# yerfor/Real3DPortrait

Measured on AMD Instinct MI355X. Metric: rendered frames/sec @ 512x512, 48 depth samples, higher is better.
Workload: dtype f32 operands as fp16 hi + lo, fp32 accumulate (SR precision 'f16mx' = the library default, superresolution.DEFAULT_SR_PRECISION; the fp32-class f16x3 is `alt_f16x3`): in block0.conv1, block1.conv0 and block1.conv1 hi*hi runs on the f16 MFMA and the two cross products on the block-scaled 8-bit MFMA

## Files before the change

### real3dportrait_amd/csrc/r3d_render.hip

```cpp

#include "r3d_common.h"
#include "r3d_stamps.h"

namespace r3d {

static constexpr int kC = R3D_FEATURES;
static constexpr int kHid = R3D_HIDDEN;
static constexpr int kOut = R3D_DECODER_OUT;
static constexpr int kWavesPerBlock = 4;

__device__ __forceinline__ void block_absmax_store(float m, float* __restrict__ absmax_part, int block_linear, float* red)
{
#pragma unroll
    for (int d = 32; d >= 1; d >>= 1) m = fmaxf(m, __shfl_xor(m, d));
    const int tid = threadIdx.y * blockDim.x + threadIdx.x, nw = (blockDim.x * blockDim.y) >> 6;
    if ((tid & 63) == 0) red[tid >> 6] = m;
    __syncthreads();
    if (tid == 0) {
        float r = red[0];
        for (int w = 1; w < nw; ++w) r = fmaxf(r, red[w]);
        absmax_part[block_linear] = r;
    }
}

// ... 506 lines not shown
#pragma unroll
    for (int ot = 0; ot < 2; ++ot) {
        uint4 a0 = L.w2f[ot][PP][0][lane], a1 = L.w2f[ot][PP][1][lane];
        const h8 wh = *reinterpret_cast<h8*>(&a0), wl = *reinterpret_cast<h8*>(&a1);
        col[ot] = __builtin_amdgcn_mfma_f32_16x16x32_f16(wl, bh, col[ot], 0, 0, 0);
        col[ot] = __builtin_amdgcn_mfma_f32_16x16x32_f16(wh, bl, col[ot], 0, 0, 0);
        col[ot] = __builtin_amdgcn_mfma_f32_16x16x32_f16(wh, bh, col[ot], 0, 0, 0);
    }
    if (PP == 1) {
        const float ys = L.ys;
        if (ys != 1.0f) {
#pragma unroll
            for (int ot = 0; ot < 2; ++ot)
#pragma unroll
                for (int r = 0; r < 4; ++r) col[ot][r] *= ys;
        }
#pragma unroll
        for (int ot = 0; ot < 2; ++ot)
#pragma unroll
            for (int r = 0; r < 4; ++r)
                col[ot][r] = __builtin_amdgcn_rcpf(1.0f + __builtin_amdgcn_exp2f(-col[ot][r])) * 1.002f - 0.001f;
    }
}

__device__ __forceinline__ void decode_tile(const DecoderLds& L, int lane, const h8 xh, const h8 xl, f32x4 (&col)[2], float& sig)
{
    DecodeState S;
    decode_a(L, lane, xh, xl, S, sig);
    decode_l2<0>(L, lane, S, col);
    decode_l2<1>(L, lane, S, col);
}

template <int CTRL, int ROW_MASK = 0xF>
__device__ __forceinline__ float dpp_f(float old, float x) {
    return __builtin_bit_cast(float, __builtin_amdgcn_update_dpp(__builtin_bit_cast(int, old), __builtin_bit_cast(int, x), CTRL, ROW_MASK, 0xF, false));
}
template <int CTRL, int ROW_MASK = 0xF>
__device__ __forceinline__ int dpp_i(int old, int x) { return __builtin_amdgcn_update_dpp(old, x, CTRL, ROW_MASK, 0xF, false); }
__device__ __forceinline__ float wave_incl_mul(float v, int) {
    v *= dpp_f<0x111>(1.0f, v); v *= dpp_f<0x112>(1.0f, v); v *= dpp_f<0x114>(1.0f, v); v *= dpp_f<0x118>(1.0f, v);
    v *= dpp_f<0x142, 0xA>(1.0f, v); v *= dpp_f<0x143, 0xC>(1.0f, v);
    return v;
}
__device__ __forceinline__ float wave_incl_add(float v, int) {
    v += dpp_f<0x111>(0.0f, v); v += dpp_f<0x112>(0.0f, v); v += dpp_f<0x114>(0.0f, v); v += dpp_f<0x118>(0.0f, v);
    v += dpp_f<0x142, 0xA>(0.0f, v); v += dpp_f<0x143, 0xC>(0.0f, v);
    return v;
}
__device__ __forceinline__ int wave_incl_add_i(int v) {
    v += dpp_i<0x111>(0, v); v += dpp_i<0x112>(0, v); v += dpp_i<0x114>(0, v); v += dpp_i<0x118>(0, v);
    v += dpp_i<0x142, 0xA>(0, v); v += dpp_i<0x143, 0xC>(0, v);
    return v;
}
__device__ __forceinline__ float wave_shift_up1(float v, float first) { return dpp_f<0x138>(first, v); }
__device__ __forceinline__ float lane63(float v) { return __builtin_bit_cast(float, __builtin_amdgcn_readlane(__builtin_bit_cast(int, v), 63)); }
__device__ __forceinline__ float wave_sum(float v) { return lane63(wave_incl_add(v, 0)); }
__device__ __forceinline__ void wave_lds_sync() {
    __builtin_amdgcn_fence(__ATOMIC_ACQ_REL, "wavefront");
    __builtin_amdgcn_wave_barrier();
}

struct XchLds { uint4 v[2][64]; };
__device__ __forceinline__ int gather_q(int lane) { return lane & 3; }
__device__ __forceinline__ int gather_s(int lane) { return lane >> 2; }
__device__ __forceinline__ void gather_to_mfma(XchLds& E, int lane, const float (&X)[8], h8& xh, h8& xl)
{
    split8_bounded(X, xh, xl);
    const int gs = lane >> 2, gq = lane & 3, q = lane >> 4, s = lane & 15;
    const int wi = 16 * gq + (gs ^ (2 * gq)), ri = 16 * q + (s ^ (2 * q));
    E.v[0][wi] = *reinterpret_cast<uint4*>(&xh);
    E.v[1][wi] = *reinterpret_cast<uint4*>(&xl);
    wave_lds_sync();
    uint4 rh = E.v[0][ri], rl = E.v[1][ri];
    wave_lds_sync();
    xh = *reinterpret_cast<h8*>(&rh);
    xl = *reinterpret_cast<h8*>(&rl);
}

template <int NS, int NCD>
struct RayLds {
    float t[NS];
    float sg[NS];
    float ts[NS];
    float ss[NS];
    float wv[NS];
    float om[NS];
    float cdf[NCD];
    int cnt[NS];
};

struct FeatLds { uint4 v[2][2 * 64]; };

typedef __amdgpu_buffer_rsrc_t PlaneRsrc;
template <int NB = 2>
struct TileGather {
    f32x4 lo[NB][4], hi[NB][4];
    float tw[NB][4];
    Tap tq[4];
    float acc[8];
    __device__ __forceinline__ void start(int H, int W, int q, float px, float py, float pz, float scale)
    {
        const float qx = px * scale, qy = py * scale, qz = pz * scale;
        const int pq = q < 2 ? q : 2;
        plane_taps(pq == 2 ? qz : qx, pq == 0 ? qy : (pq == 1 ? qz : qx), H, W, pq * H * W * 8, tq);
#pragma unroll
        for (int k = 0; k < 4; ++k) tq[k].idx *= 16;
    }
    template <int P, int B>
    __device__ __forceinline__ void issue(const PlaneRsrc rsrc, unsigned qoff)
    {
#pragma unroll
        for (int k = 0; k < 4; ++k) {
            const int wbits = __builtin_bit_cast(int, tq[k].w);
            const unsigned off = (unsigned)(P == 0 ? __builtin_amdgcn_mov_dpp(tq[k].idx, 0x00, 0xF, 0xF, true) : P == 1 ? __builtin_amdgcn_mov_dpp(tq[k].idx, 0x55, 0xF, 0xF, true) : __builtin_amdgcn_mov_dpp(tq[k].idx, 0xAA, 0xF, 0xF, true)) + qoff;
            tw[B][k] = __builtin_bit_cast(float, P == 0 ? __builtin_amdgcn_mov_dpp(wbits, 0x00, 0xF, 0xF, true) : P == 1 ? __builtin_amdgcn_mov_dpp(wbits, 0x55, 0xF, 0xF, true) : __builtin_amdgcn_mov_dpp(wbits, 0xAA, 0xF, 0xF, true));
            lo[B][k] = __builtin_bit_cast(f32x4, __builtin_amdgcn_raw_buffer_load_b128(rsrc, (int)off, 0, 0));
            hi[B][k] = __builtin_bit_cast(f32x4, __builtin_amdgcn_raw_buffer_load_b128(rsrc, (int)(off + 16u), 0, 0));
        }
    }
    template <int B>
    __device__ __forceinline__ void pin(f32x4& d0, f32x4& d1)
    {
        asm volatile("" : "+v"(lo[B][0]), "+v"(lo[B][1]), "+v"(lo[B][2]), "+v"(lo[B][3]), "+v"(hi[B][0]), "+v"(hi[B][1]), "+v"(hi[B][2]), "+v"(hi[B][3]),
                          "+v"(d0), "+v"(d1));
    }
    template <int P, int B>
    __device__ __forceinline__ void consume()
    {
        float pa[8];
#pragma unroll
        for (int c = 0; c < 8; ++c) pa[c] = 0.0f;
#pragma unroll
        for (int k = 0; k < 4; ++k) {
            const float w = tw[B][k];
            const f32x4 a4 = lo[B][k], b4 = hi[B][k];
            pa[0] += a4[0] * w; pa[1] += a4[1] * w; pa[2] += a4[2] * w; pa[3] += a4[3] * w;
            pa[4] += b4[0] * w; pa[5] += b4[1] * w; pa[6] += b4[2] * w; pa[7] += b4[3] * w;
        }
#pragma unroll
        for (int c = 0; c < 8; ++c) acc[c] = P == 0 ? pa[c] : acc[c] + pa[c];
    }
    __device__ __forceinline__ void finish(FeatLds& F, int slot, int wi, float xs3)
    {
        float X[8];
#pragma unroll
        for (int c = 0; c < 8; ++c) X[c] = acc[c] * xs3;
        h8 xh, xl;
        split8_bounded(X, xh, xl);
        F.v[0][slot * 64 + wi] = *reinterpret_cast<uint4*>(&xh);
        F.v[1][slot * 64 + wi] = *reinterpret_cast<uint4*>(&xl);
    }
};

template <int NT, int GPF, bool TRI, int NB = 2, typename DepthFn, typename FirstFn>
__device__ __forceinline__ void decode_pass(FeatLds& F, const DecoderLds& dec, const float4* __restrict__ P, int H, int W, int D, int lane,
                                            float ox, float oy, float oz, float dx, float dy, float dz, float scale, float xs3,
                                            DepthFn depth_of, FirstFn first_done, f32x4 (&col0)[NT], f32x4 (&col1)[NT], float (&sig)[NT], f32x4* gp = nullptr)
{
    const int gq = lane & 3, gs = lane >> 2, q = lane >> 4, s = lane & 15;
    const int wi = 16 * gq + (gs ^ (2 * gq)), ri = 16 * q + (s ^ (2 * q));
    const uint64_t pb = (uint64_t)(uintptr_t)P;
    void* pu = reinterpret_cast<void*>((uintptr_t)(((uint64_t)(unsigned)__builtin_amdgcn_readfirstlane((int)(pb >> 32)) << 32) |
                                                   (unsigned)__builtin_amdgcn_readfirstlane((int)(pb & 0xffffffffu))));
    const PlaneRsrc pl = __builtin_amdgcn_make_buffer_rsrc(pu, 0, __builtin_amdgcn_readfirstlane(3 * (TRI ? D : 1) * H * W * 128), 0x00020000);
    const unsigned qoff = 32u * (unsigned)gq;
    TileGather<NB> g;
    auto gather_whole = [&](int t) {
        const float tg = depth_of(t);
        if constexpr (TRI) {
            float X[8]; h8 xh, xl;
            gather_sample<GPF, true>(P, H, W, gq, ox + tg * dx, oy + tg * dy, oz + tg * dz, scale, xs3, X, D);
            split8_bounded(X, xh, xl);
            F.v[0][(t & 1) * 64 + wi] = *reinterpret_cast<uint4*>(&xh); F.v[1][(t & 1) * 64 + wi] = *reinterpret_cast<uint4*>(&xl);
        } else {
            f32x4 z0 = {0.f, 0.f, 0.f, 0.f}, z1 = z0;
            g.start(H, W, gq, ox + tg * dx, oy + tg * dy, oz + tg * dz, scale);
            g.template issue<0, 0>(pl, qoff);
            if constexpr (NB == 2) {
                g.template issue<1, 1>(pl, qoff);
                g.template pin<0>(z0, z1); g.template consume<0, 0>();
                g.template issue<2, 0>(pl, qoff);
                g.template pin<1>(z0, z1); g.template consume<1, 1>();
                g.template pin<0>(z0, z1); g.template consume<2, 0>();
            } else {
                g.template pin<0>(z0, z1); g.template consume<0, 0>();
                g.template issue<1, 0>(pl, qoff);
                g.template pin<0>(z0, z1); g.template consume<1, 0>();
                g.template issue<2, 0>(pl, qoff);
                g.template pin<0>(z0, z1); g.template consume<2, 0>();
            }
            g.finish(F, t & 1, wi, xs3);
        }
    };
    gather_whole(0);
    first_done();
#pragma unroll
    for (int t = 0; t < NT; ++t) {
        wave_lds_sync();
        uint4 rh = F.v[0][(t & 1) * 64 + ri], rl4 = F.v[1][(t & 1) * 64 + ri];
        const h8 xh = *reinterpret_cast<h8*>(&rh), xl = *reinterpret_cast<h8*>(&rl4);
        const bool more = t + 1 < NT;
        DecodeState S;
        f32x4 c2[2];
        if (more && !TRI) {
            const float tg = depth_of(t + 1);
            g.start(H, W, gq, ox + tg * dx, oy + tg * dy, oz + tg * dz, scale);
            g.template issue<0, 0>(pl, qoff);
        }
        __builtin_amdgcn_sched_barrier(0);
        decode_a(dec, lane, xh, xl, S, sig[t]);
        __builtin_amdgcn_sched_barrier(0);
        if (more && !TRI) { g.template pin<0>(S.h[0], S.h[3]); g.template consume<0, 0>(); g.template issue<1, 0>(pl, qoff); }
        __builtin_amdgcn_sched_barrier(0);
        decode_l2<0>(dec, lane, S, c2);
        __builtin_amdgcn_sched_barrier(0);
        if (more && !TRI) { g.template pin<0>(c2[0], c2[1]); g.template consume<1, 0>(); g.template issue<2, 0>(pl, qoff); }
        __builtin_amdgcn_sched_barrier(0);
        decode_l2<1>(dec, lane, S, c2);
        __builtin_amdgcn_sched_barrier(0);
        if (more && !TRI) { g.template pin<0>(c2[0], c2[1]); g.template consume<2, 0>(); g.finish(F, (t + 1) & 1, wi, xs3); }
        if (more && TRI) gather_whole(t + 1);
        if (gp) { gp[(2 * t) * 64] = c2[0]; gp[(2 * t + 1) * 64] = c2[1]; }
        else { col0[t] = c2[0]; col1[t] = c2[1]; }
        __builtin_amdgcn_sched_barrier(0);
    }
}

template <int SLOTS>
__device__ __forceinline__ void march(const float* T, const float* S, float* wv, int n, int lane,
                                      float& wsum, float& dsum)
{
    float carry = 1.0f, ws = 0.0f, ds = 0.0f;
#pragma unroll
    for (int sl = 0; sl < SLOTS; ++sl) {
        const int i = sl * 64 + lane;
        const bool act = i < n - 1;
        const int i0 = act ? i : 0;
        const float t0 = T[i0], t1 = T[i0 + 1], s0 = S[i0], s1 = S[i0 + 1];
        const float delta = t1 - t0;
        const float dmid = (s0 + s1) * 0.5f;
        const float tmid = (t0 + t1) * 0.5f;
        const float sp = softplus20(dmid - 1.0f);
        const float alpha = one_minus_exp_neg(sp * delta);
        const float om1 = act ? (1.0f - alpha + 1e-10f) : 1.0f;
        const float incl = wave_incl_mul(om1, lane);
        const float excl = wave_shift_up1(incl, 1.0f);
        const float w = act ? alpha * (carry * excl) : 0.0f;
        carry *= lane63(incl);
        if (act) wv[i] = w;
        ws += w;
        ds += w * tmid;
    }
    wsum = wave_sum(ws);
    dsum = wave_sum(ds);
}

struct RenderArgs {
    const float4* planes4; int N, H, W, M, D;
    const float* w1; const float* b1; const float* w2; const float* b2;
    const float* origins; const float* dirs;
    const float* cam_c2w; const float* cam_K; int cam_R;
    uint2* split_out; const float* split_scale; size_t split_scale_stride;
    const float* ray_start; const float* ray_end; const uint8_t* valid;
    int* gstate; int nlimit_blocks;
    int Nc, Nf; float scale; int white_back;
    const float* noise_c; const float* u_f; unsigned long long seed;
    const DecFold* fold;
    float* rgb; float* depth; float* wsum; int rgb_cm;
    unsigned long long* clk;
    f32x4* park_g;
};

struct RayIter {
    int strips, n, c, row, sa, sb, sc, R, strip, N, M, col0;
    long long lin, lstride, nrays;
    __device__ __forceinline__ void init(const RenderArgs& a, int R_, int wave)
    {
        const int wv = __builtin_amdgcn_readfirstlane(wave);
        R = R_; N = a.N; M = a.M;
        strips = (R > 0 && (R & 7) == 0 && (gridDim.x & 7) == 0) ? 1 : 0;
        if (strips) {
            const unsigned xcd = blockIdx.x & 7, bx = blockIdx.x >> 3, nbx = gridDim.x >> 3;
            strip = R >> 3; col0 = (int)xcd * strip;
            const unsigned per_img = (unsigned)strip * (unsigned)R;
            const unsigned w0 = bx * kWavesPerBlock + (unsigned)wv, st = nbx * kWavesPerBlock;
            n = (int)(w0 / per_img); const unsigned rem = w0 - (unsigned)n * per_img;
            c = (int)(rem / (unsigned)R); row = (int)(rem - (unsigned)c * (unsigned)R);
            sa = (int)(st / per_img); const unsigned srem = st - (unsigned)sa * per_img;
            sb = (int)(srem / (unsigned)R); sc = (int)(srem - (unsigned)sb * (unsigned)R);
        } else {
            nrays = (long long)a.N * a.M;
            lin = (long long)blockIdx.x * kWavesPerBlock + wv;
            lstride = (long long)gridDim.x * kWavesPerBlock;
        }
    }
    __device__ __forceinline__ bool get(int& ray, int& img) const
    {
        if (strips) { if (n >= N) return false; img = n; ray = n * M + row * R + col0 + c; return true; }
        if (lin >= nrays) return false;
        ray = (int)lin; img = ray / M; return true;
    }
    __device__ __forceinline__ void advance()
    {
        if (strips) {
            row += sc; if (row >= R) { row -= R; ++c; }
            c += sb;   if (c >= strip) { c -= strip; ++n; }
            n += sa;
        } else lin += lstride;
    }
};

template <int NTC, int NTF, int OCC, int GPF, bool TRI = false>
__global__ __launch_bounds__(256, OCC) void render_kernel(RenderArgs a, int R)
{
    constexpr int SLOTS = (16 * (NTC + NTF) + 63) / 64;
    constexpr int CSLOTS = (16 * NTC + 63) / 64;
    constexpr int FSLOTS = NTF > 0 ? (16 * NTF + 63) / 64 : 1;
    typedef RayLds<16 * (NTC + NTF) + 8, 16 * NTC + 8> RayL;
    __shared__ __attribute__((aligned(16))) DecoderLds dec;
    __shared__ __attribute__((aligned(16))) RayL rl[kWavesPerBlock];
    __shared__ __attribute__((aligned(16))) FeatLds feat[kWavesPerBlock];
    constexpr bool PARK = NTF > 0 && NTC <= 3;
    constexpr bool GPARK = NTF > 0 && NTC > 3;
    __shared__ __attribute__((aligned(16))) f32x4 park[PARK ? kWavesPerBlock : 1][PARK ? 2 * NTC : 1][64];

    stage_decoder(dec, a.w1, a.b1, a.w2, a.b2, a.fold);
    __syncthreads();
    const float xs3 = dec.xs3;

    const int lane = threadIdx.x & 63, wave = threadIdx.x >> 6;
    const int q = lane >> 4, s = lane & 15;
    const int gs = gather_s(lane);
    RayL& L = rl[wave];
    FeatLds& F = feat[wave];
    int pmin = 0x7fffffff, pmax = (int)0x80000000, pany = 0;
    for (int b = lane; b < a.nlimit_blocks; b += 64) {
        const int* p = a.gstate + kStateHeader + 3 * b;
        pmin = min(pmin, p[0]); pmax = max(pmax, p[1]); pany |= p[2];
    }
#pragma unroll
    for (int d = 32; d >= 1; d >>= 1) { pmin = min(pmin, __shfl_xor(pmin, d)); pmax = max(pmax, __shfl_xor(pmax, d)); pany |= __shfl_xor(pany, d); }
    const float gmin_start = ord2f(pmin), gmax_start = ord2f(pmax);
    const bool any_valid = pany != 0;
    const int Nc_all = a.Nc;
    float run_min = INFINITY, run_max = -INFINITY;
    R3D_STAMP_DECL;
    int st_rays_ = 0; (void)st_rays_;
    if (blockIdx.x == (gridDim.x >> 1) && threadIdx.x == 0) clk_begin(kernarg_clk<RenderArgs>());

    RayIter it;
    it.init(a, R, wave);
    for (;; it.advance()) {
        typedef const __attribute__((address_space(4))) RenderArgs* KArgs;
        KArgs ap = (KArgs)__builtin_amdgcn_kernarg_segment_ptr();
        asm volatile("" : "+s"(ap));
        const auto& A = *ap;
        const int Nc = NTF > 0 ? A.Nc : Nc_all, Nf = A.Nf, S = Nc + Nf;
        int ray, n;
        if (!it.get(ray, n)) break;
        ++st_rays_;
        R3D_STAMP(7);
        const float4* P = A.planes4 + (size_t)n * 3 * (TRI ? A.D : 1) * A.H * A.W * 8;
        float ox, oy, oz, dx, dy, dz;
        if (A.cam_c2w) {
            float o3[3], d3[3];
            make_ray(A.cam_c2w + 16 * n, A.cam_K + 9 * n, A.cam_R, ray - n * A.M, o3, d3);
            ox = o3[0]; oy = o3[1]; oz = o3[2]; dx = d3[0]; dy = d3[1]; dz = d3[2];
        } else {
            ox = A.origins[3 * (size_t)ray]; oy = A.origins[3 * (size_t)ray + 1]; oz = A.origins[3 * (size_t)ray + 2];
            dx = A.dirs[3 * (size_t)ray]; dy = A.dirs[3 * (size_t)ray + 1]; dz = A.dirs[3 * (size_t)ray + 2];
        }
        float start = A.ray_start[ray], end = A.ray_end[ray];
        if (!A.valid[ray] && any_valid) { start = gmin_start; end = gmax_start; }

        const float span = end - start;
        const float delta = span / (float)(Nc - 1);
        float tc[NTC];
#pragma unroll
        for (int nt = 0; nt < NTC; ++nt) {
            const int k = 16 * nt + s;
            const bool act = k < Nc;
            const float step = (float)k / (float)(Nc - 1);
            float u = 0.0f;
            if (act) u = A.noise_c ? A.noise_c[(size_t)ray * Nc + k] : hash_uniform(A.seed, 0, (uint64_t)ray * Nc + k);
            tc[nt] = act ? (start + step * span) + u * delta : start;
        }
        R3D_STAMP(0);
        f32x4 colc[2][NTC];
        float sigc[NTC];
        f32x4* gpark = nullptr;
        if constexpr (GPARK) gpark = A.park_g + ((size_t)(blockIdx.x * kWavesPerBlock + wave) * (2 * (NTC + NTF))) * 64 + lane;
        {
            if (q == 0) {
#pragma unroll
                for (int nt = 0; nt < NTC; ++nt) {
                    const int k = 16 * nt + s;
                    if (k < Nc) L.t[k] = tc[nt];
                }
            }
            wave_lds_sync();
            auto dof = [&](int t) { const int k = 16 * t + gs; return k < Nc ? L.t[k] : start; };
            decode_pass<NTC, GPF, TRI, (OCC >= 3 ? 1 : 2)>(F, dec, P, A.H, A.W, A.D, lane, ox, oy, oz, dx, dy, dz, A.scale, xs3, dof,
                                                           [&]() { R3D_STAMP(8); }, colc[0], colc[1], sigc, gpark);
        }
        constexpr bool parked = PARK;
        if (parked) {
#pragma unroll
            for (int nt = 0; nt < NTC; ++nt) { park[PARK ? wave : 0][PARK ? 2 * nt : 0][lane] = colc[0][nt]; park[PARK ? wave : 0][PARK ? 2 * nt + 1 : 0][lane] = colc[1][nt]; }
        }

        if (q == 0) {
#pragma unroll
            for (int nt = 0; nt < NTC; ++nt) {
                const int k = 16 * nt + s;
                if (k < Nc) L.sg[k] = sigc[nt];
            }
        }
        wave_lds_sync();
        R3D_STAMP(1);

        float wsum, dsum;
        f32x4 colf[2][NTF > 0 ? NTF : 1];
        bool fine_done = false;
        if constexpr (NTF > 0) { if (Nf > 0) {
            fine_done = true;
            march<CSLOTS>(L.t, L.sg, L.wv, Nc, lane, wsum, dsum);
            wave_lds_sync();
            const int ns = Nc - 3;
            float omega[CSLOTS], tot = 0.0f;
#pragma unroll
            for (int sl = 0; sl < CSLOTS; ++sl) {
                const int i = sl * 64 + lane;
                const bool act = i < ns;
                const int i0 = act ? i : 0;
                const float w0 = L.wv[i0], w1v = L.wv[i0 + 1], w2v = L.wv[i0 + 2];
                const float sv = (fmaxf(w0, w1v) + fmaxf(w1v, w2v)) * 0.5f + 0.01f;
                omega[sl] = act ? sv + 1e-5f : 0.0f;
                tot += omega[sl];
            }
            tot = wave_sum(tot);
            float carry = 0.0f;
            if (lane == 0) L.cdf[0] = 0.0f;
#pragma unroll
            for (int sl = 0; sl < CSLOTS; ++sl) {
                const int i = sl * 64 + lane;
                const float incl = wave_incl_add(omega[sl] / tot, lane);
                if (i < ns) L.cdf[i + 1] = carry + incl;
                carry += lane63(incl);
            }
            wave_lds_sync();
#pragma unroll
            for (int sl = 0; sl < FSLOTS; ++sl) {
                const int j = sl * 64 + lane;
                if (j < Nf) {
                    const float u = A.u_f ? A.u_f[(size_t)ray * Nf + j] : hash_uniform(A.seed, 1, (uint64_t)ray * Nf + j);
                    int lo = 0, hi = ns + 1;
                    while (lo < hi) { const int mid = (lo + hi) >> 1; if (L.cdf[mid] <= u) lo = mid + 1; else hi = mid; }
                    const int below = max(lo - 1, 0), above = min(lo, ns);
                    const float cb = L.cdf[below], ca = L.cdf[above];
                    const float bb = 0.5f * (L.t[below] + L.t[below + 1]);
                    const float ba = 0.5f * (L.t[above] + L.t[above + 1]);
                    float den = ca - cb;
                    if (den < 1e-5f) den = 1.0f;
                    L.t[Nc + j] = bb + (u - cb) / den * (ba - bb);
                }
            }
            wave_lds_sync();
            R3D_STAMP(2);
            float sigf[NTF > 0 ? NTF : 1];
            {
                auto dof = [&](int t) { const int k = 16 * t + gs; return L.t[Nc + (k < Nf ? k : 0)]; };
                decode_pass<(NTF > 0 ? NTF : 1), GPF, TRI, (OCC >= 3 ? 1 : 2)>(F, dec, P, A.H, A.W, A.D, lane, ox, oy, oz, dx, dy, dz, A.scale, xs3, dof,
                                                                             [&]() { R3D_STAMP(9); }, colf[0], colf[1], sigf, GPARK ? gpark + 2 * NTC * 64 : nullptr);
            }
            if (q == 0) {
#pragma unroll
                for (int nt = 0; nt < NTF; ++nt) {
                    const int k = 16 * nt + s;
                    if (k < Nf) L.sg[Nc + k] = sigf[nt];
                }
            }
            wave_lds_sync();
            R3D_STAMP(3);
            int rank[SLOTS];
            bool fast = true;
#pragma unroll
            for (int sl = 0; sl < CSLOTS; ++sl) {
                const int i = sl * 64 + lane;
                const bool act = i < Nc - 1;
                fast = fast && (!act || L.t[act ? i : 0] <= L.t[act ? i + 1 : 0]);
            }
            fast = __all(fast);
            if (fast) {
#pragma unroll
                for (int sl = 0; sl < CSLOTS + 1; ++sl) { const int i = sl * 64 + lane; if (i <= Nc) L.cnt[i] = 0; }
                wave_lds_sync();
                int rf[FSLOTS];
#pragma unroll
                for (int sl = 0; sl < FSLOTS; ++sl) {
                    const int j = sl * 64 + lane;
                    const bool act = j < Nf;
                    const float tj = L.t[Nc + (act ? j : 0)];
                    int lo = 0, hi = Nc;
                    while (lo < hi) { const int mid = (lo + hi) >> 1; if (L.t[mid] <= tj) lo = mid + 1; else hi = mid; }
                    int f = 0;
                    for (int k = 0; k < Nf; ++k) f += (L.t[Nc + k] < tj) ? 1 : 0;
                    rf[sl] = lo + f;
                    if (act) atomicAdd(&L.cnt[lo], 1);
                }
                wave_lds_sync();
                int carry = 0;
                int rc[CSLOTS];
#pragma unroll
                for (int sl = 0; sl < CSLOTS; ++sl) {
                    const int i = sl * 64 + lane;
                    int v = i < Nc ? L.cnt[i] : 0;
                    v = wave_incl_add_i(v);
                    rc[sl] = i + carry + v;
                    carry += __builtin_amdgcn_readlane(v, 63);
                }
                wave_lds_sync();
#pragma unroll
                for (int sl = 0; sl < CSLOTS; ++sl) { const int i = sl * 64 + lane; if (i < Nc) L.cnt[rc[sl]] = i; }
#pragma unroll
                for (int sl = 0; sl < FSLOTS; ++sl) { const int j = sl * 64 + lane; if (j < Nf) L.cnt[rf[sl]] = Nc + j; }
                wave_lds_sync();
                bool ok = true;
#pragma unroll
                for (int sl = 0; sl < CSLOTS; ++sl) { const int i = sl * 64 + lane; if (i < Nc) ok = ok && L.cnt[rc[sl]] == i; }
#pragma unroll
                for (int sl = 0; sl < FSLOTS; ++sl) { const int j = sl * 64 + lane; if (j < Nf) ok = ok && L.cnt[rf[sl]] == Nc + j; }
                fast = __all(ok);
                if (fast) {
#pragma unroll
                    for (int sl = 0; sl < CSLOTS; ++sl) { const int i = sl * 64 + lane; if (i < Nc) L.cnt[i] = rc[sl]; }
#pragma unroll
                    for (int sl = 0; sl < FSLOTS; ++sl) { const int j = sl * 64 + lane; if (j < Nf) L.cnt[Nc + j] = rf[sl]; }
                    wave_lds_sync();
#pragma unroll
                    for (int sl = 0; sl < SLOTS; ++sl) {
                        const int i = sl * 64 + lane;
                        rank[sl] = L.cnt[i < S ? i : 0];
                    }
                }
            }
            if (!fast) {
                if (lane == 0) atomicAdd(&g_merge_fallbacks, 1u);
#pragma unroll
                for (int sl = 0; sl < SLOTS; ++sl) {
                    const int i = sl * 64 + lane;
                    const float ti = L.t[i < S ? i : 0];
                    int cnt = 0;
                    for (int j = 0; j < S; ++j) {
                        const float tj = L.t[j];
                        cnt += (tj < ti || (tj == ti && j < i)) ? 1 : 0;
                    }
                    rank[sl] = cnt;
                }
            }
#pragma unroll
            for (int sl = 0; sl < SLOTS; ++sl) {
                const int i = sl * 64 + lane;
                if (i < S) { L.ts[rank[sl]] = L.t[i]; L.ss[rank[sl]] = L.sg[i]; }
            }
            wave_lds_sync();
            R3D_STAMP(4);
            march<SLOTS>(L.ts, L.ss, L.wv, S, lane, wsum, dsum);
            wave_lds_sync();
#pragma unroll
            for (int sl = 0; sl < SLOTS; ++sl) {
                const int i = sl * 64 + lane, r = rank[sl];
                if (i < S) {
                    const float wl = r > 0 ? L.wv[r - 1] : 0.0f;
                    const float wr = r < S - 1 ? L.wv[r] : 0.0f;
                    L.om[i] = 0.5f * (wl + wr);
                }
            }
        } }
        if (!fine_done) {
            march<CSLOTS>(L.t, L.sg, L.wv, Nc, lane, wsum, dsum);
            wave_lds_sync();
#pragma unroll
            for (int sl = 0; sl < CSLOTS; ++sl) {
                const int i = sl * 64 + lane;
                if (i < Nc) {
                    const float wl = i > 0 ? L.wv[i - 1] : 0.0f;
                    const float wr = i < Nc - 1 ? L.wv[i] : 0.0f;
                    L.om[i] = 0.5f * (wl + wr);
                }
            }
        }
        wave_lds_sync();
        R3D_STAMP(5);

        f32x4 acc[2];
        acc[0] = (f32x4){0.f, 0.f, 0.f, 0.f};
        acc[1] = acc[0];
#pragma unroll
        for (int nt = 0; nt < NTC; ++nt) {
            const int k = 16 * nt + s;
            const float om = k < Nc ? L.om[k] : 0.0f;
            f32x4 cc0 = colc[0][nt], cc1 = colc[1][nt];
            if (parked) { cc0 = park[PARK ? wave : 0][PARK ? 2 * nt : 0][lane]; cc1 = park[PARK ? wave : 0][PARK ? 2 * nt + 1 : 0][lane]; }
            if constexpr (GPARK) { cc0 = gpark[(2 * nt) * 64]; cc1 = gpark[(2 * nt + 1) * 64]; }
            acc[0] += cc0 * om;
            acc[1] += cc1 * om;
        }
        if constexpr (NTF > 0) {
#pragma unroll
            for (int nt = 0; nt < NTF; ++nt) {
                const int k = 16 * nt + s;
                const float om = (fine_done && k < Nf) ? L.om[Nc + k] : 0.0f;
                f32x4 cf0 = colf[0][nt], cf1 = colf[1][nt];
                if constexpr (GPARK) { cf0 = gpark[(2 * (NTC + nt)) * 64]; cf1 = gpark[(2 * (NTC + nt) + 1) * 64]; }
                acc[0] += cf0 * om;
                acc[1] += cf1 * om;
            }
        }
#pragma unroll
        for (int ot = 0; ot < 2; ++ot)
#pragma unroll
            for (int r = 0; r < 4; ++r) {
                float v = acc[ot][r];
                v += dpp_f<0x128>(0.0f, v); v += dpp_f<0x124>(0.0f, v); v += dpp_f<0x122>(0.0f, v); v += dpp_f<0x121>(0.0f, v);
                if (A.white_back) v = v + 1.0f - wsum;
                acc[ot][r] = v * 2.0f - 1.0f;
            }
        if (s == 0 && A.split_out) {
            const float* sc = A.split_scale + (size_t)n * A.split_scale_stride;
            const size_t pix = (size_t)(ray - n * A.M), plane = (size_t)(kC / 8) * A.M;
#pragma unroll
            for (int ot = 0; ot < 2; ++ot) {
                const float4 s4 = *reinterpret_cast<const float4*>(sc + 16 * ot + 4 * q);
                const float sv[4] = {s4.x, s4.y, s4.z, s4.w};
                typedef _Float16 h4v __attribute__((ext_vector_type(4)));
                h4v hi, lo;
#pragma unroll
                for (int r = 0; r < 4; ++r) {
                    _Float16 hh, ll;
                    split_scaled(acc[ot][r], sv[r], hh, ll);
                    hi[r] = hh; lo[r] = ll;
                }
                uint2* dst = A.split_out + (((size_t)n * 2 * plane + (size_t)(2 * ot + (q >> 1)) * A.M + pix) * 2 + (q & 1));
                dst[0] = *reinterpret_cast<uint2*>(&hi);
                dst[2 * plane] = *reinterpret_cast<uint2*>(&lo);
            }
        }
        if (s == 0) {
            if (A.rgb_cm) {
                float* o = A.rgb + ((size_t)n * kC + 4 * q) * A.M + (ray - n * A.M);
#pragma unroll
                for (int r = 0; r < 4; ++r) { o[(size_t)r * A.M] = acc[0][r]; o[(size_t)(16 + r) * A.M] = acc[1][r]; }
            } else {
                float4* o4 = reinterpret_cast<float4*>(A.rgb + (size_t)ray * kC);
                o4[q] = make_float4(acc[0][0], acc[0][1], acc[0][2], acc[0][3]);
                o4[4 + q] = make_float4(acc[1][0], acc[1][1], acc[1][2], acc[1][3]);
            }
        }
        float lmin = INFINITY, lmax = -INFINITY;
#pragma unroll
        for (int sl = 0; sl < SLOTS; ++sl) {
            const int i = sl * 64 + lane;
            if (i < S) { const float v = L.t[i]; lmin = fminf(lmin, v); lmax = fmaxf(lmax, v); }
        }
        run_min = fminf(run_min, lmin); run_max = fmaxf(run_max, lmax);
        if (lane == 0) {
            if (A.depth) A.depth[ray] = dsum / wsum;
            A.wsum[ray] = wsum;
        }
        wave_lds_sync();
        R3D_STAMP(6);
    }
    R3D_STAMP_FLUSH(10, st_rays_);
    if (blockIdx.x == (gridDim.x >> 1) && threadIdx.x == 0) clk_end(kernarg_clk<RenderArgs>());
#pragma unroll
    for (int d = 32; d >= 1; d >>= 1) {
        run_min = fminf(run_min, __shfl_xor(run_min, d));
        run_max = fmaxf(run_max, __shfl_xor(run_max, d));
    }
    if (lane == 0 && run_min <= run_max) {
        atomicMin(&a.gstate[3], f2ord(run_min));
        atomicMax(&a.gstate[4], f2ord(run_max));
    }
}

template <bool TRI>
__global__ __launch_bounds__(256, 2) void run_model_kernel(const float4* __restrict__ planes4, int N, int H, int W, int D,
                                                          const float* w1, const float* b1, const float* w2, const float* b2,
                                                          const float* __restrict__ coords, int npts, float scale,
                                                          float* __restrict__ rgb, float* __restrict__ sigma, const DecFold* __restrict__ fold)
{
    __shared__ __attribute__((aligned(16))) DecoderLds dec;
    __shared__ __attribute__((aligned(16))) XchLds xch[kWavesPerBlock];
    stage_decoder(dec, w1, b1, w2, b2, fold);
    __syncthreads();
    const float xs3 = dec.xs3;
    const int lane = threadIdx.x & 63, wave = threadIdx.x >> 6;
    const int q = lane >> 4, s = lane & 15;
    const int gq = gather_q(lane), gs = gather_s(lane);
    XchLds& E = xch[wave];
    const long long total = (long long)N * npts;
    const long long chunks = (total + 63) / 64;
    for (long long ch = (long long)blockIdx.x * kWavesPerBlock + wave; ch < chunks; ch += (long long)gridDim.x * kWavesPerBlock) {
        long long idx[4];
        f32x4 col[2][4];
        float sig[4];
#pragma unroll
        for (int nt = 0; nt < 4; ++nt) {
            idx[nt] = ch * 64 + 16 * nt + s;
            const long long ig = ch * 64 + 16 * nt + gs;
            const long long ii = ig < total ? ig : total - 1;
            const int n = (int)(ii / npts);
            const float4* P = planes4 + (size_t)n * 3 * (TRI ? D : 1) * H * W * 8;
            float X[8];
            f32x4 c2[2];
            h8 xh, xl;
            gather_sample<3, TRI>(P, H, W, gq, coords[3 * ii], coords[3 * ii + 1], coords[3 * ii + 2], scale, xs3, X, D);
            gather_to_mfma(E, lane, X, xh, xl);
            decode_tile(dec, lane, xh, xl, c2, sig[nt]);
            col[0][nt] = c2[0]; col[1][nt] = c2[1];
            __builtin_amdgcn_sched_barrier(0);
        }
#pragma unroll
        for (int nt = 0; nt < 4; ++nt) {
            if (idx[nt] < total) {
                float4* o4 = reinterpret_cast<float4*>(rgb + (size_t)idx[nt] * kC);
                o4[q] = make_float4(col[0][nt][0], col[0][nt][1], col[0][nt][2], col[0][nt][3]);
                o4[4 + q] = make_float4(col[1][nt][0], col[1][nt][1], col[1][nt][2], col[1][nt][3]);
                if (q == 0) sigma[idx[nt]] = sig[nt];
            }
        }
    }
}

static inline size_t render_state_bytes(size_t nrays) { return ((kStateHeader + 3 * ((nrays + kLimitsBlock - 1) / kLimitsBlock)) * sizeof(int) + 63) & ~(size_t)63; }
static constexpr size_t kFoldBytes = 64 + kAbsmaxBlocks * sizeof(float);
static constexpr int kMaxGrid = 512;

static const DecFold* launch_decoder_fold(const float* planes_nhwc, size_t plane_floats, const float* plane_absmax, int n_plane_absmax,
                                          const float* w1, const float* b1, const float* w2, void* fold_mem, hipStream_t st)
{
    DecFold* fold = reinterpret_cast<DecFold*>(fold_mem);
    float* part = reinterpret_cast<float*>(reinterpret_cast<char*>(fold_mem) + 64);
    if (!plane_absmax || n_plane_absmax <= 0) {
        hipLaunchKernelGGL(plane_absmax_kernel, dim3(kAbsmaxBlocks), dim3(256), 0, st, reinterpret_cast<const float4*>(planes_nhwc), plane_floats / 4, part);
        plane_absmax = part; n_plane_absmax = kAbsmaxBlocks;
    }
    hipLaunchKernelGGL(decoder_fold_kernel, dim3(1), dim3(256), 0, st, plane_absmax, n_plane_absmax, w1, b1, w2, fold);
    return fold;
}

template <int NTC, int NTF>
static void launch_render(const RenderArgs& a, int R, int grid, hipStream_t st)
{
    hipLaunchKernelGGL((render_kernel<NTC, NTF, 2, 1>), dim3(grid), dim3(256), 0, st, a, R);
}


template <int NTC, int NTF>
static void launch_render_tri(const RenderArgs& a, int R, int grid, hipStream_t st)
{
    hipLaunchKernelGGL((render_kernel<NTC, NTF, 2, 3, true>), dim3(grid), dim3(256), 0, st, a, R);
}

}

using namespace r3d;

R3D_STAMP_READER(r3d_debug_stamps)

static inline bool nhwc32_fast_path(const void* a, const void* b, const void* c, int C, int HW, int depth, int add_flip)
{
    const bool aligned16 = !(((uintptr_t)a | (uintptr_t)b | (uintptr_t)c) & 15);
    return C == 32 && depth == 1 && add_flip == 0 && (HW & 63) == 0 && aligned16;
}
extern "C" size_t r3d_planes_absmax_partials(int N, int C, int H, int W, int depth)
{
    if (N <= 0 || C <= 0 || H <= 0 || W <= 0 || depth < 1) return 0;
    const size_t HW = (size_t)H * W;
    return ((HW + 31) / 32) * ((C + 31) / 32) * (size_t)N * 3 * depth;
}

extern "C" int r3d_planes_to_nhwc(const float* planes_nchw, const float* add_nchw, float* planes_nhwc,
                                  int N, int C, int H, int W, int depth, int add_flip, float* absmax_partials, int* n_partials,
                                  r3d_stream_t stream)
{
    if (absmax_partials && !n_partials) { set_error("planes_to_nhwc: absmax_partials needs n_partials"); return R3D_ERR_INVALID_ARG; }
    if (!planes_nchw || !planes_nhwc || N <= 0 || C <= 0 || H <= 0 || W <= 0 || depth < 1 || depth > 16 || add_flip < 0 || add_flip > 63) {
        set_error("planes_to_nhwc: bad argument"); return R3D_ERR_INVALID_ARG;
    }
    const int HW = H * W;
    dim3 grid((HW + 31) / 32, (C + 31) / 32, N * 3 * depth), block(32, 8);
    ProfScope ps(R3D_PROF_LAYOUT, (hipStream_t)stream);
    if (nhwc32_fast_path(planes_nchw, add_nchw, planes_nhwc, C, HW, depth, add_flip)) {
        if (n_partials) *n_partials = (HW / 64) * N * 3;
        hipLaunchKernelGGL(planes_to_nhwc32_kernel, dim3(HW / 64, N * 3), dim3(256), 0, (hipStream_t)stream, planes_nchw, add_nchw, planes_nhwc, HW, absmax_partials);
        return check_launch("planes_to_nhwc");
    }
    if (n_partials) *n_partials = (int)(grid.x * grid.y * grid.z);
    hipLaunchKernelGGL(planes_to_nhwc_kernel, grid, block, 0, (hipStream_t)stream, planes_nchw, add_nchw, planes_nhwc, C, HW, W, add_flip, depth, absmax_partials);
    return check_launch("planes_to_nhwc");
}

extern "C" int r3d_raygen(const float* c2w, const float* intrinsics, int N, int R,
                          float* origins, float* dirs, r3d_stream_t stream)
{
    if (!c2w || !intrinsics || !origins || !dirs || N <= 0 || R <= 0) { set_error("raygen: bad argument"); return R3D_ERR_INVALID_ARG; }
    dim3 grid((R * R + 255) / 256, N);
    ProfScope ps(R3D_PROF_MISC, (hipStream_t)stream);
    hipLaunchKernelGGL(raygen_kernel, grid, dim3(256), 0, (hipStream_t)stream, c2w, intrinsics, R, origins, dirs);
    return check_launch("raygen");
}

static int render_grid(size_t nrays)
{
    const size_t max_blocks = ((nrays + kWavesPerBlock - 1) / kWavesPerBlock + 7) / 8 * 8;
    return max_blocks < (size_t)kMaxGrid ? (int)max_blocks : kMaxGrid;
}
static bool render_parks(int Nc, int Nf) { return (Nc > 48 || Nf > 48) && Nf > 0; }
static size_t render_park_bytes(size_t nrays, int Nc, int Nf) { return render_parks(Nc, Nf) ? (size_t)render_grid(nrays) * kWavesPerBlock * 24 * 64 * sizeof(f32x4) : 0; }

extern "C" size_t r3d_render_workspace_bytes(int N, int M, int Nc, int Nf)
{
    const size_t nrays = (size_t)N * M;
    return render_state_bytes(nrays) + 2 * nrays * sizeof(float) + 64 + kFoldBytes + render_park_bytes(nrays, Nc, Nf);
}
// ... 130 lines not shown
```

### real3dportrait_amd/csrc/r3d_stamps.h

```cpp
#pragma once
#ifdef R3D_STAMPS
namespace r3d { static __device__ unsigned long long g_stamps[32]; }
#define R3D_STAMP_DECL unsigned long long st_acc_[12] = {0, 0, 0, 0, 0, 0, 0, 0, 0, 0, 0, 0}; const unsigned long long st_r0_ = wall_clock64(); \
                       unsigned long long st_t_ = clock64(); const unsigned long long st_c0_ = st_t_
#define R3D_STAMP_CLOCKS(slot) do { if ((threadIdx.x & 63) == 0) { atomicAdd(&r3d::g_stamps[slot], clock64() - st_c0_); atomicAdd(&r3d::g_stamps[(slot) + 1], wall_clock64() - st_r0_); } } while (0)
#define R3D_STAMP(i) do { const unsigned long long n_ = clock64(); st_acc_[i] += n_ - st_t_; st_t_ = n_; } while (0)
#define R3D_STAMP_FLUSH(nphase, units) do { R3D_STAMP_CLOCKS(28); if ((threadIdx.x & 63) == 0) { for (int i_ = 0; i_ < (nphase); ++i_) atomicAdd(&r3d::g_stamps[i_], st_acc_[i_]); \
                                                atomicAdd(&r3d::g_stamps[31], (unsigned long long)(units)); } } while (0)
#define R3D_STAMP_READER(name) extern "C" int name(unsigned long long* host) { \
    if (hipMemcpyFromSymbol(host, HIP_SYMBOL(r3d::g_stamps), sizeof(unsigned long long) * 32) != hipSuccess) return -1; \
    unsigned long long z[32] = {}; return hipMemcpyToSymbol(HIP_SYMBOL(r3d::g_stamps), z, sizeof(z)) == hipSuccess ? 0 : -1; }
#else
#define R3D_STAMP_DECL do { } while (0)
#define R3D_STAMP(i) do { } while (0)
#define R3D_STAMP_FLUSH(nphase, units) do { } while (0)
#define R3D_STAMP_CLOCKS(slot) do { } while (0)
#define R3D_STAMP_READER(name)
#endif
```

Measured before the change: 1809.

## Prefetch next ray header and overlap merge-rank with first fine gather

Restructures the render loop so the next ray's start/end, origin/dir, validity and noise values are loaded during the tail of the current ray, with ray setup finished at loop end. The coarse/fine merge ranking moves into a callback that runs under the latency of the first fine-pass gather loads, and split-scale loads are hoisted early. The binary search gets a fixed unrolled trip count, and a few uniform values are made scalar via readfirstlane. This adds register pressure from the prefetched header state and more profiling stamp slots.

New measurement: 1815 (median of 6 runs). Within noise of the previous version (+0.3%).

```diff
diff --git a/real3dportrait_amd/csrc/r3d_render.hip b/real3dportrait_amd/csrc/r3d_render.hip
--- a/real3dportrait_amd/csrc/r3d_render.hip
+++ b/real3dportrait_amd/csrc/r3d_render.hip
@@ -682,10 +682,10 @@
     }
 };
 
-template <int NT, int GPF, bool TRI, int NB = 2, typename DepthFn, typename FirstFn>
+template <int NT, int GPF, bool TRI, int NB = 2, typename DepthFn, typename FirstFn, typename UnderFn>
 __device__ __forceinline__ void decode_pass(FeatLds& F, const DecoderLds& dec, const float4* __restrict__ P, int H, int W, int D, int lane,
                                             float ox, float oy, float oz, float dx, float dy, float dz, float scale, float xs3,
-                                            DepthFn depth_of, FirstFn first_done, f32x4 (&col0)[NT], f32x4 (&col1)[NT], float (&sig)[NT], f32x4* gp = nullptr)
+                                            DepthFn depth_of, FirstFn first_evt, UnderFn under_first, f32x4 (&col0)[NT], f32x4 (&col1)[NT], float (&sig)[NT], f32x4* gp = nullptr)
 {
     const int gq = lane & 3, gs = lane >> 2, q = lane >> 4, s = lane & 15;
     const int wi = 16 * gq + (gs ^ (2 * gq)), ri = 16 * q + (s ^ (2 * q));
@@ -697,6 +697,7 @@
     TileGather<NB> g;
     auto gather_whole = [&](int t) {
         const float tg = depth_of(t);
+        if constexpr (TRI || NB != 2) { if (t == 0) { under_first(); first_evt(1); } }
         if constexpr (TRI) {
             float X[8]; h8 xh, xl;
             gather_sample<GPF, true>(P, H, W, gq, ox + tg * dx, oy + tg * dy, oz + tg * dz, scale, xs3, X, D);
@@ -705,13 +706,22 @@
         } else {
             f32x4 z0 = {0.f, 0.f, 0.f, 0.f}, z1 = z0;
             g.start(H, W, gq, ox + tg * dx, oy + tg * dy, oz + tg * dz, scale);
+            if (t == 0) first_evt(4);
             g.template issue<0, 0>(pl, qoff);
             if constexpr (NB == 2) {
                 g.template issue<1, 1>(pl, qoff);
-                g.template pin<0>(z0, z1); g.template consume<0, 0>();
-                g.template issue<2, 0>(pl, qoff);
-                g.template pin<1>(z0, z1); g.template consume<1, 1>();
-                g.template pin<0>(z0, z1); g.template consume<2, 0>();
+                if (t == 0) {
+                    first_evt(0);
+                    __builtin_amdgcn_sched_barrier(0); under_first(); __builtin_amdgcn_sched_barrier(0);
+                    first_evt(1);
+                }
+                g.template pin<0>(z0, z1); if (t == 0) first_evt(2);
+                g.template consume<0, 0>();
+                g.template issue<2, 0>(pl, qoff); if (t == 0) first_evt(3);
+                g.template pin<1>(z0, z1); if (t == 0) first_evt(2);
+                g.template consume<1, 1>(); if (t == 0) first_evt(3);
+                g.template pin<0>(z0, z1); if (t == 0) first_evt(2);
+                g.template consume<2, 0>();
             } else {
                 g.template pin<0>(z0, z1); g.template consume<0, 0>();
                 g.template issue<1, 0>(pl, qoff);
@@ -723,7 +733,7 @@
         }
     };
     gather_whole(0);
-    first_done();
+    first_evt(3);
 #pragma unroll
     for (int t = 0; t < NT; ++t) {
         wave_lds_sync();
@@ -856,7 +866,7 @@
 
     stage_decoder(dec, a.w1, a.b1, a.w2, a.b2, a.fold);
     __syncthreads();
-    const float xs3 = dec.xs3;
+    const float xs3 = __builtin_bit_cast(float, __builtin_amdgcn_readfirstlane(__builtin_bit_cast(int, dec.xs3)));
 
     const int lane = threadIdx.x & 63, wave = threadIdx.x >> 6;
     const int q = lane >> 4, s = lane & 15;
@@ -870,6 +880,7 @@
     }
 #pragma unroll
     for (int d = 32; d >= 1; d >>= 1) { pmin = min(pmin, __shfl_xor(pmin, d)); pmax = max(pmax, __shfl_xor(pmax, d)); pany |= __shfl_xor(pany, d); }
+    pmin = __builtin_amdgcn_readfirstlane(pmin); pmax = __builtin_amdgcn_readfirstlane(pmax); pany = __builtin_amdgcn_readfirstlane(pany);
     const float gmin_start = ord2f(pmin), gmax_start = ord2f(pmax);
     const bool any_valid = pany != 0;
     const int Nc_all = a.Nc;
@@ -880,58 +891,103 @@
 
     RayIter it;
     it.init(a, R, wave);
-    for (;; it.advance()) {
-        typedef const __attribute__((address_space(4))) RenderArgs* KArgs;
+    typedef const __attribute__((address_space(4))) RenderArgs* KArgs;
+    int ray = 0, n = 0;
+    bool have_ray = false;
+    float ox = 0.f, oy = 0.f, oz = 0.f, dx = 0.f, dy = 0.f, dz = 0.f, start = 0.f;
+    int h_ray = 0, h_n = 0;
+    bool h_ok = false;
+    float h_start = 0.f, h_end = 0.f, h_o[3] = {0.f, 0.f, 0.f}, h_d[3] = {0.f, 0.f, 0.f}, h_u[NTC];
+    uint8_t h_valid = 0;
+    auto next_head_issue = [&]() {
+        KArgs hp = (KArgs)__builtin_amdgcn_kernarg_segment_ptr();
+        asm volatile("" : "+s"(hp));
+        const auto& A = *hp;
+        const int Nc = NTF > 0 ? A.Nc : Nc_all;
+        h_ok = it.get(h_ray, h_n);
+        h_start = h_end = 0.0f; h_valid = 0;
+#pragma unroll
+        for (int c = 0; c < 3; ++c) h_o[c] = h_d[c] = 0.0f;
+#pragma unroll
+        for (int nt = 0; nt < NTC; ++nt) h_u[nt] = 0.0f;
+        if (h_ok) {
+            h_start = A.ray_start[h_ray]; h_end = A.ray_end[h_ray]; h_valid = A.valid[h_ray];
+            if (!A.cam_c2w) {
+                h_o[0] = A.origins[3 * (size_t)h_ray]; h_o[1] = A.origins[3 * (size_t)h_ray + 1]; h_o[2] = A.origins[3 * (size_t)h_ray + 2];
+                h_d[0] = A.dirs[3 * (size_t)h_ray]; h_d[1] = A.dirs[3 * (size_t)h_ray + 1]; h_d[2] = A.dirs[3 * (size_t)h_ray + 2];
+            }
+            if (A.noise_c) {
+#pragma unroll
+                for (int nt = 0; nt < NTC; ++nt) {
+                    const int k = 16 * nt + s;
+                    if (k < Nc) h_u[nt] = A.noise_c[(size_t)h_ray * Nc + k];
+                }
+            }
+        }
+    };
+    auto next_head_finish = [&]() {
+        have_ray = h_ok;
+        if (h_ok) {
+            KArgs hp = (KArgs)__builtin_amdgcn_kernarg_segment_ptr();
+            asm volatile("" : "+s"(hp));
+            const auto& A = *hp;
+            const int Nc = NTF > 0 ? A.Nc : Nc_all;
+            ray = h_ray; n = h_n;
+            if (A.cam_c2w) {
+                float o3[3], d3[3];
+                make_ray(A.cam_c2w + 16 * n, A.cam_K + 9 * n, A.cam_R, ray - n * A.M, o3, d3);
+                ox = o3[0]; oy = o3[1]; oz = o3[2]; dx = d3[0]; dy = d3[1]; dz = d3[2];
+            } else {
+                ox = h_o[0]; oy = h_o[1]; oz = h_o[2]; dx = h_d[0]; dy = h_d[1]; dz = h_d[2];
+            }
+            auto uni = [](float v) { return __builtin_bit_cast(float, __builtin_amdgcn_readfirstlane(__builtin_bit_cast(int, v))); };
+            ox = uni(ox); oy = uni(oy); oz = uni(oz); dx = uni(dx); dy = uni(dy); dz = uni(dz);
+            float end = h_end;
+            start = h_start;
+            if (!h_valid && any_valid) { start = gmin_start; end = gmax_start; }
+            start = uni(start); end = uni(end);
+            const float span = end - start;
+            const float delta = span / (float)(Nc - 1);
+            float tc[NTC];
+#pragma unroll
+            for (int nt = 0; nt < NTC; ++nt) {
+                const int k = 16 * nt + s;
+                const bool act = k < Nc;
+                const float step = (float)k / (float)(Nc - 1);
+                float u = 0.0f;
+                if (act) u = A.noise_c ? h_u[nt] : hash_uniform(A.seed, 0, (uint64_t)ray * Nc + k);
+                tc[nt] = act ? (start + step * span) + u * delta : start;
+            }
+            if (q == 0) {
+#pragma unroll
+                for (int nt = 0; nt < NTC; ++nt) {
+                    const int k = 16 * nt + s;
+                    if (k < Nc) L.t[k] = tc[nt];
+                }
+            }
+        }
+        wave_lds_sync();
+    };
+    next_head_issue();
+    next_head_finish();
+    R3D_STAMP(0);
+    while (have_ray) {
         KArgs ap = (KArgs)__builtin_amdgcn_kernarg_segment_ptr();
         asm volatile("" : "+s"(ap));
         const auto& A = *ap;
         const int Nc = NTF > 0 ? A.Nc : Nc_all, Nf = A.Nf, S = Nc + Nf;
-        int ray, n;
-        if (!it.get(ray, n)) break;
         ++st_rays_;
         R3D_STAMP(7);
         const float4* P = A.planes4 + (size_t)n * 3 * (TRI ? A.D : 1) * A.H * A.W * 8;
-        float ox, oy, oz, dx, dy, dz;
-        if (A.cam_c2w) {
-            float o3[3], d3[3];
-            make_ray(A.cam_c2w + 16 * n, A.cam_K + 9 * n, A.cam_R, ray - n * A.M, o3, d3);
-            ox = o3[0]; oy = o3[1]; oz = o3[2]; dx = d3[0]; dy = d3[1]; dz = d3[2];
-        } else {
-            ox = A.origins[3 * (size_t)ray]; oy = A.origins[3 * (size_t)ray + 1]; oz = A.origins[3 * (size_t)ray + 2];
-            dx = A.dirs[3 * (size_t)ray]; dy = A.dirs[3 * (size_t)ray + 1]; dz = A.dirs[3 * (size_t)ray + 2];
-        }
-        float start = A.ray_start[ray], end = A.ray_end[ray];
-        if (!A.valid[ray] && any_valid) { start = gmin_start; end = gmax_start; }
-
-        const float span = end - start;
-        const float delta = span / (float)(Nc - 1);
-        float tc[NTC];
-#pragma unroll
-        for (int nt = 0; nt < NTC; ++nt) {
-            const int k = 16 * nt + s;
-            const bool act = k < Nc;
-            const float step = (float)k / (float)(Nc - 1);
-            float u = 0.0f;
-            if (act) u = A.noise_c ? A.noise_c[(size_t)ray * Nc + k] : hash_uniform(A.seed, 0, (uint64_t)ray * Nc + k);
-            tc[nt] = act ? (start + step * span) + u * delta : start;
-        }
-        R3D_STAMP(0);
         f32x4 colc[2][NTC];
         float sigc[NTC];
         f32x4* gpark = nullptr;
         if constexpr (GPARK) gpark = A.park_g + ((size_t)(blockIdx.x * kWavesPerBlock + wave) * (2 * (NTC + NTF))) * 64 + lane;
         {
-            if (q == 0) {
-#pragma unroll
-                for (int nt = 0; nt < NTC; ++nt) {
-                    const int k = 16 * nt + s;
-                    if (k < Nc) L.t[k] = tc[nt];
-                }
-            }
-            wave_lds_sync();
             auto dof = [&](int t) { const int k = 16 * t + gs; return k < Nc ? L.t[k] : start; };
             decode_pass<NTC, GPF, TRI, (OCC >= 3 ? 1 : 2)>(F, dec, P, A.H, A.W, A.D, lane, ox, oy, oz, dx, dy, dz, A.scale, xs3, dof,
-                                                           [&]() { R3D_STAMP(8); }, colc[0], colc[1], sigc, gpark);
+                                                           [&](int e) { if (e == 0) R3D_STAMP(8); else if (e == 2) R3D_STAMP(10); else if (e == 3) R3D_STAMP(12); else if (e == 4) R3D_STAMP(16); },
+                                                           []() {}, colc[0], colc[1], sigc, gpark);
         }
         constexpr bool parked = PARK;
         if (parked) {
@@ -952,6 +1008,14 @@
         float wsum, dsum;
         f32x4 colf[2][NTF > 0 ? NTF : 1];
         bool fine_done = false;
+        float4 ssc[2] = {make_float4(0.f, 0.f, 0.f, 0.f), make_float4(0.f, 0.f, 0.f, 0.f)};
+        auto load_split_scale = [&]() {
+            if (A.split_out) {
+                const float* sc = A.split_scale + (size_t)n * A.split_scale_stride;
+                ssc[0] = *reinterpret_cast<const float4*>(sc + 4 * q);
+                ssc[1] = *reinterpret_cast<const float4*>(sc + 16 + 4 * q);
+            }
+        };
         if constexpr (NTF > 0) { if (Nf > 0) {
             fine_done = true;
             march<CSLOTS>(L.t, L.sg, L.wv, Nc, lane, wsum, dsum);
@@ -997,11 +1061,93 @@
             }
             wave_lds_sync();
             R3D_STAMP(2);
+            auto merge_ranks = [&]() {
+                bool fast = true;
+#pragma unroll
+                for (int sl = 0; sl < CSLOTS; ++sl) {
+                    const int i = sl * 64 + lane;
+                    const bool act = i < Nc - 1;
+                    fast = fast && (!act || L.t[act ? i : 0] <= L.t[act ? i + 1 : 0]);
+                }
+                fast = __all(fast);
+                if (fast) {
+#pragma unroll
+                    for (int sl = 0; sl < CSLOTS + 1; ++sl) { const int i = sl * 64 + lane; if (i <= Nc) L.cnt[i] = 0; }
+                    wave_lds_sync();
+                    int rf[FSLOTS];
+#pragma unroll
+                    for (int sl = 0; sl < FSLOTS; ++sl) {
+                        const int j = sl * 64 + lane;
+                        const bool act = j < Nf;
+                        const float tj = L.t[Nc + (act ? j : 0)];
+                        int lo = 0, hi = Nc;
+#pragma unroll
+                        for (int n = 16 * NTC; n > 0; n >>= 1) {
+                            const int mid = (lo + hi) >> 1;
+                            const bool go = lo < hi, le = L.t[mid] <= tj;
+                            lo = (go && le) ? mid + 1 : lo;
+                            hi = (go && !le) ? mid : hi;
+                        }
+                        int f = 0;
+                        for (int k = 0; k < Nf; ++k) f += (L.t[Nc + k] < tj) ? 1 : 0;
+                        rf[sl] = lo + f;
+                        if (act) atomicAdd(&L.cnt[lo], 1);
+                    }
+                    wave_lds_sync();
+                    int carry = 0;
+                    int rc[CSLOTS];
+#pragma unroll
+                    for (int sl = 0; sl < CSLOTS; ++sl) {
+                        const int i = sl * 64 + lane;
+                        int v = i < Nc ? L.cnt[i] : 0;
+                        v = wave_incl_add_i(v);
+                        rc[sl] = i + carry + v;
+                        carry += __builtin_amdgcn_readlane(v, 63);
+                    }
+                    wave_lds_sync();
+#pragma unroll
+                    for (int sl = 0; sl < CSLOTS; ++sl) { const int i = sl * 64 + lane; if (i < Nc) L.cnt[rc[sl]] = i; }
+#pragma unroll
+                    for (int sl = 0; sl < FSLOTS; ++sl) { const int j = sl * 64 + lane; if (j < Nf) L.cnt[rf[sl]] = Nc + j; }
+                    wave_lds_sync();
+                    bool ok = true;
+#pragma unroll
+                    for (int sl = 0; sl < CSLOTS; ++sl) { const int i = sl * 64 + lane; if (i < Nc) ok = ok && L.cnt[rc[sl]] == i; }
+#pragma unroll
+                    for (int sl = 0; sl < FSLOTS; ++sl) { const int j = sl * 64 + lane; if (j < Nf) ok = ok && L.cnt[rf[sl]] == Nc + j; }
+                    fast = __all(ok);
+                    if (fast) {
+#pragma unroll
+                        for (int sl = 0; sl < CSLOTS; ++sl) { const int i = sl * 64 + lane; if (i < Nc) L.cnt[i] = rc[sl]; }
+#pragma unroll
+                        for (int sl = 0; sl < FSLOTS; ++sl) { const int j = sl * 64 + lane; if (j < Nf) L.cnt[Nc + j] = rf[sl]; }
+                    }
+                }
+                if (!fast) {
+                    if (lane == 0) atomicAdd(&g_merge_fallbacks, 1u);
+                    int rk[SLOTS];
+#pragma unroll
+                    for (int sl = 0; sl < SLOTS; ++sl) {
+                        const int i = sl * 64 + lane;
+                        const float ti = L.t[i < S ? i : 0];
+                        int cnt = 0;
+                        for (int j = 0; j < S; ++j) {
+                            const float tj = L.t[j];
+                            cnt += (tj < ti || (tj == ti && j < i)) ? 1 : 0;
+                        }
+                        rk[sl] = cnt;
+                    }
+#pragma unroll
+                    for (int sl = 0; sl < SLOTS; ++sl) { const int i = sl * 64 + lane; if (i < S) L.cnt[i] = rk[sl]; }
+                }
+                wave_lds_sync();
+            };
             float sigf[NTF > 0 ? NTF : 1];
             {
                 auto dof = [&](int t) { const int k = 16 * t + gs; return L.t[Nc + (k < Nf ? k : 0)]; };
                 decode_pass<(NTF > 0 ? NTF : 1), GPF, TRI, (OCC >= 3 ? 1 : 2)>(F, dec, P, A.H, A.W, A.D, lane, ox, oy, oz, dx, dy, dz, A.scale, xs3, dof,
-                                                                             [&]() { R3D_STAMP(9); }, colf[0], colf[1], sigf, GPARK ? gpark + 2 * NTC * 64 : nullptr);
+                                                                             [&](int e) { if (e == 0) R3D_STAMP(9); else if (e == 1) R3D_STAMP(14); else if (e == 2) R3D_STAMP(11); else if (e == 3) R3D_STAMP(13); else R3D_STAMP(17); },
+                                                                             merge_ranks, colf[0], colf[1], sigf, GPARK ? gpark + 2 * NTC * 64 : nullptr);
             }
             if (q == 0) {
 #pragma unroll
@@ -1012,82 +1158,13 @@
             }
             wave_lds_sync();
             R3D_STAMP(3);
+            it.advance();
+            next_head_issue();
+            R3D_STAMP(15);
+            load_split_scale();
             int rank[SLOTS];
-            bool fast = true;
-#pragma unroll
-            for (int sl = 0; sl < CSLOTS; ++sl) {
-                const int i = sl * 64 + lane;
-                const bool act = i < Nc - 1;
-                fast = fast && (!act || L.t[act ? i : 0] <= L.t[act ? i + 1 : 0]);
-            }
-            fast = __all(fast);
-            if (fast) {
-#pragma unroll
-                for (int sl = 0; sl < CSLOTS + 1; ++sl) { const int i = sl * 64 + lane; if (i <= Nc) L.cnt[i] = 0; }
-                wave_lds_sync();
-                int rf[FSLOTS];
-#pragma unroll
-                for (int sl = 0; sl < FSLOTS; ++sl) {
-                    const int j = sl * 64 + lane;
-                    const bool act = j < Nf;
-                    const float tj = L.t[Nc + (act ? j : 0)];
-                    int lo = 0, hi = Nc;
-                    while (lo < hi) { const int mid = (lo + hi) >> 1; if (L.t[mid] <= tj) lo = mid + 1; else hi = mid; }
-                    int f = 0;
-                    for (int k = 0; k < Nf; ++k) f += (L.t[Nc + k] < tj) ? 1 : 0;
-                    rf[sl] = lo + f;
-                    if (act) atomicAdd(&L.cnt[lo], 1);
-                }
-                wave_lds_sync();
-                int carry = 0;
-                int rc[CSLOTS];
-#pragma unroll
-                for (int sl = 0; sl < CSLOTS; ++sl) {
-                    const int i = sl * 64 + lane;
-                    int v = i < Nc ? L.cnt[i] : 0;
-                    v = wave_incl_add_i(v);
-                    rc[sl] = i + carry + v;
-                    carry += __builtin_amdgcn_readlane(v, 63);
-                }
-                wave_lds_sync();
-#pragma unroll
-                for (int sl = 0; sl < CSLOTS; ++sl) { const int i = sl * 64 + lane; if (i < Nc) L.cnt[rc[sl]] = i; }
-#pragma unroll
-                for (int sl = 0; sl < FSLOTS; ++sl) { const int j = sl * 64 + lane; if (j < Nf) L.cnt[rf[sl]] = Nc + j; }
-                wave_lds_sync();
-                bool ok = true;
-#pragma unroll
-                for (int sl = 0; sl < CSLOTS; ++sl) { const int i = sl * 64 + lane; if (i < Nc) ok = ok && L.cnt[rc[sl]] == i; }
-#pragma unroll
-                for (int sl = 0; sl < FSLOTS; ++sl) { const int j = sl * 64 + lane; if (j < Nf) ok = ok && L.cnt[rf[sl]] == Nc + j; }
-                fast = __all(ok);
-                if (fast) {
-#pragma unroll
-                    for (int sl = 0; sl < CSLOTS; ++sl) { const int i = sl * 64 + lane; if (i < Nc) L.cnt[i] = rc[sl]; }
-#pragma unroll
-                    for (int sl = 0; sl < FSLOTS; ++sl) { const int j = sl * 64 + lane; if (j < Nf) L.cnt[Nc + j] = rf[sl]; }
-                    wave_lds_sync();
-#pragma unroll
-                    for (int sl = 0; sl < SLOTS; ++sl) {
-                        const int i = sl * 64 + lane;
-                        rank[sl] = L.cnt[i < S ? i : 0];
-                    }
-                }
-            }
-            if (!fast) {
-                if (lane == 0) atomicAdd(&g_merge_fallbacks, 1u);
-#pragma unroll
-                for (int sl = 0; sl < SLOTS; ++sl) {
-                    const int i = sl * 64 + lane;
-                    const float ti = L.t[i < S ? i : 0];
-                    int cnt = 0;
-                    for (int j = 0; j < S; ++j) {
-                        const float tj = L.t[j];
-                        cnt += (tj < ti || (tj == ti && j < i)) ? 1 : 0;
-                    }
-                    rank[sl] = cnt;
-                }
-            }
+#pragma unroll
+            for (int sl = 0; sl < SLOTS; ++sl) { const int i = sl * 64 + lane; rank[sl] = L.cnt[i < S ? i : 0]; }
 #pragma unroll
             for (int sl = 0; sl < SLOTS; ++sl) {
                 const int i = sl * 64 + lane;
@@ -1108,6 +1185,10 @@
             }
         } }
         if (!fine_done) {
+            it.advance();
+            next_head_issue();
+            R3D_STAMP(15);
+            load_split_scale();
             march<CSLOTS>(L.t, L.sg, L.wv, Nc, lane, wsum, dsum);
             wave_lds_sync();
 #pragma unroll
@@ -1157,11 +1238,10 @@
                 acc[ot][r] = v * 2.0f - 1.0f;
             }
         if (s == 0 && A.split_out) {
-            const float* sc = A.split_scale + (size_t)n * A.split_scale_stride;
             const size_t pix = (size_t)(ray - n * A.M), plane = (size_t)(kC / 8) * A.M;
 #pragma unroll
             for (int ot = 0; ot < 2; ++ot) {
-                const float4 s4 = *reinterpret_cast<const float4*>(sc + 16 * ot + 4 * q);
+                const float4 s4 = ssc[ot];
                 const float sv[4] = {s4.x, s4.y, s4.z, s4.w};
                 typedef _Float16 h4v __attribute__((ext_vector_type(4)));
                 h4v hi, lo;
@@ -1200,8 +1280,10 @@
         }
         wave_lds_sync();
         R3D_STAMP(6);
-    }
-    R3D_STAMP_FLUSH(10, st_rays_);
+        next_head_finish();
+        R3D_STAMP(0);
+    }
+    R3D_STAMP_FLUSH(18, st_rays_);
     if (blockIdx.x == (gridDim.x >> 1) && threadIdx.x == 0) clk_end(kernarg_clk<RenderArgs>());
 #pragma unroll
     for (int d = 32; d >= 1; d >>= 1) {
diff --git a/real3dportrait_amd/csrc/r3d_stamps.h b/real3dportrait_amd/csrc/r3d_stamps.h
--- a/real3dportrait_amd/csrc/r3d_stamps.h
+++ b/real3dportrait_amd/csrc/r3d_stamps.h
@@ -1,7 +1,7 @@
 #pragma once
 #ifdef R3D_STAMPS
 namespace r3d { static __device__ unsigned long long g_stamps[32]; }
-#define R3D_STAMP_DECL unsigned long long st_acc_[12] = {0, 0, 0, 0, 0, 0, 0, 0, 0, 0, 0, 0}; const unsigned long long st_r0_ = wall_clock64(); \
+#define R3D_STAMP_DECL unsigned long long st_acc_[18] = {0, 0, 0, 0, 0, 0, 0, 0, 0, 0, 0, 0, 0, 0, 0, 0, 0, 0}; const unsigned long long st_r0_ = wall_clock64(); \
                        unsigned long long st_t_ = clock64(); const unsigned long long st_c0_ = st_t_
 #define R3D_STAMP_CLOCKS(slot) do { if ((threadIdx.x & 63) == 0) { atomicAdd(&r3d::g_stamps[slot], clock64() - st_c0_); atomicAdd(&r3d::g_stamps[(slot) + 1], wall_clock64() - st_r0_); } } while (0)
 #define R3D_STAMP(i) do { const unsigned long long n_ = clock64(); st_acc_[i] += n_ - st_t_; st_t_ = n_; } while (0)
```
